# ioloizou/g1_locomotion

Hardware: AMD Instinct MI355X
Metric: QP solves/sec, SRBD N=10 12-state/12-input (higher is better)
Workload: dtype f64; 1 GPU; configs[1]: batch=4096/GPU random SRBD states, N=10, 2-contact alternating single support friction cone, fp64; tails deferred (SRBDQP_FLAG_DEFER_TAIL: the ~4 % of a batch that reach a rho-restart mark finish in the next launch on their stream; srbdqp_flush inside the timed region, every batch complete when the clock stops); steps rotate over 4 distinct device batches; horizon=10, batch_per_gpu=4096, kernel=wave_defer_f64_n10_s2, streams=2, longest_first_hint=False, deferred_tails=True, world_size=1, distinct_batches=4, max_iter=250, rho_restart_iter=0, rho_restart_count=0, set_up_dtype=f64

## Files before the change

### g1_locomotion_amd/csrc/srbdqp_admm.hpp

```cpp
#pragma once
#include "srbdqp_common.hpp"

namespace srbdqp {

#ifdef SRBDQP_PROFILE_ADMM
#define ADMM_T(var) do { unsigned long long t_; asm volatile("s_memtime %0\n\ts_waitcnt lgkmcnt(0)" : "=s"(t_) :: "memory"); var = (long long)t_; } while (0)
#else
#define ADMM_T(var) do { } while (0)
#endif

__device__ __forceinline__ double dpp_swap1(double v) {
    int lo = __double2loint(v), hi = __double2hiint(v);
    lo = __builtin_amdgcn_update_dpp(lo, lo, 0xB1, 0xF, 0xF, false);
    hi = __builtin_amdgcn_update_dpp(hi, hi, 0xB1, 0xF, 0xF, false);
    return __hiloint2double(hi, lo);
}

__device__ __forceinline__ double dpp_swap2(double v) {
    int lo = __double2loint(v), hi = __double2hiint(v);
    lo = __builtin_amdgcn_update_dpp(lo, lo, 0x4E, 0xF, 0xF, false);
    hi = __builtin_amdgcn_update_dpp(hi, hi, 0x4E, 0xF, 0xF, false);
    return __hiloint2double(hi, lo);
}

__device__ __forceinline__ int wave_next(int v) { return __builtin_amdgcn_update_dpp(0, v, 0x130, 0xF, 0xF, true); }
__device__ __forceinline__ int wave_prev(int v) { return __builtin_amdgcn_update_dpp(0, v, 0x138, 0xF, 0xF, true); }
__device__ __forceinline__ float wave_next(float v) { return __int_as_float(wave_next(__float_as_int(v))); }
__device__ __forceinline__ float wave_prev(float v) { return __int_as_float(wave_prev(__float_as_int(v))); }
__device__ __forceinline__ double wave_next(double v) { return __hiloint2double(wave_next(__double2hiint(v)), wave_next(__double2loint(v))); }
__device__ __forceinline__ double wave_prev(double v) { return __hiloint2double(wave_prev(__double2hiint(v)), wave_prev(__double2loint(v))); }
template <typename T> __device__ __forceinline__ T contact_fz(T v, int ax) { const T n1 = wave_next(v), n2 = wave_next(n1); return (ax == 0) ? n2 : ((ax == 1) ? n1 : v); }
template <typename T> __device__ __forceinline__ T contact_sum_xy(T v) { const T p1 = wave_prev(v), p2 = wave_prev(p1); return p2 + p1; }

typedef unsigned v2u_t __attribute__((ext_vector_type(2)));
__device__ __forceinline__ void row_chunks(int v, int (&ch)[4]) {
    const v2u_t ab = __builtin_amdgcn_permlane32_swap((unsigned)v, (unsigned)v, false, false);
    const v2u_t p = __builtin_amdgcn_permlane16_swap(ab[0], ab[0], false, false);
    const v2u_t q = __builtin_amdgcn_permlane16_swap(ab[1], ab[1], false, false);
    ch[0] = (int)p[0]; ch[1] = (int)p[1]; ch[2] = (int)q[0]; ch[3] = (int)q[1];
}
__device__ __forceinline__ void row_chunks(double v, double (&ch)[4]) {
    int lo[4], hi[4];
    row_chunks(__double2loint(v), lo);
    row_chunks(__double2hiint(v), hi);
#pragma unroll
    for (int c = 0; c < 4; ++c) ch[c] = __hiloint2double(hi[c], lo[c]);
}

__device__ __forceinline__ double bperm_f64(double v, int src_lane) {
    const int lo = __builtin_amdgcn_ds_bpermute(src_lane << 2, __double2loint(v));
    const int hi = __builtin_amdgcn_ds_bpermute(src_lane << 2, __double2hiint(v));
    return __hiloint2double(hi, lo);
}

#define SRBDQP_FD(A, K, J) "v_fmac_f64_dpp %" #A ", %4, %" #K " row_newbcast:" #J " row_mask:0xf bank_mask:0xf\n\t"
#define SRBDQP_FD4(K0, K1, K2, K3, J0, J1, J2, J3) SRBDQP_FD(0, K0, J0) SRBDQP_FD(1, K1, J1) SRBDQP_FD(2, K2, J2) SRBDQP_FD(3, K3, J3)
template <int CNT>
__device__ __forceinline__ void fmac_row_bcast_block(double (&acc)[4], double ch, const double* k) {
    static_assert(CNT == 4 || CNT == 8 || CNT == 12 || CNT == 16, "whole groups of four terms");
    if constexpr (CNT == 4)
        asm volatile("s_nop 1\n\t" SRBDQP_FD4(5, 6, 7, 8, 0, 1, 2, 3)
                     : "+v"(acc[0]), "+v"(acc[1]), "+v"(acc[2]), "+v"(acc[3]) : "v"(ch), "v"(k[0]), "v"(k[1]), "v"(k[2]), "v"(k[3]));
    else if constexpr (CNT == 8)
        asm volatile("s_nop 1\n\t" SRBDQP_FD4(5, 6, 7, 8, 0, 1, 2, 3) SRBDQP_FD4(9, 10, 11, 12, 4, 5, 6, 7)
                     : "+v"(acc[0]), "+v"(acc[1]), "+v"(acc[2]), "+v"(acc[3])
                     : "v"(ch), "v"(k[0]), "v"(k[1]), "v"(k[2]), "v"(k[3]), "v"(k[4]), "v"(k[5]), "v"(k[6]), "v"(k[7]));
    else if constexpr (CNT == 12)
        asm volatile("s_nop 1\n\t" SRBDQP_FD4(5, 6, 7, 8, 0, 1, 2, 3) SRBDQP_FD4(9, 10, 11, 12, 4, 5, 6, 7) SRBDQP_FD4(13, 14, 15, 16, 8, 9, 10, 11)
                     : "+v"(acc[0]), "+v"(acc[1]), "+v"(acc[2]), "+v"(acc[3])
                     : "v"(ch), "v"(k[0]), "v"(k[1]), "v"(k[2]), "v"(k[3]), "v"(k[4]), "v"(k[5]), "v"(k[6]), "v"(k[7]), "v"(k[8]), "v"(k[9]), "v"(k[10]),
                       "v"(k[11]));
    else
        asm volatile("s_nop 1\n\t" SRBDQP_FD4(5, 6, 7, 8, 0, 1, 2, 3) SRBDQP_FD4(9, 10, 11, 12, 4, 5, 6, 7) SRBDQP_FD4(13, 14, 15, 16, 8, 9, 10, 11)
                     SRBDQP_FD4(17, 18, 19, 20, 12, 13, 14, 15)
                     : "+v"(acc[0]), "+v"(acc[1]), "+v"(acc[2]), "+v"(acc[3])
                     : "v"(ch), "v"(k[0]), "v"(k[1]), "v"(k[2]), "v"(k[3]), "v"(k[4]), "v"(k[5]), "v"(k[6]), "v"(k[7]), "v"(k[8]), "v"(k[9]), "v"(k[10]),
                       "v"(k[11]), "v"(k[12]), "v"(k[13]), "v"(k[14]), "v"(k[15]));
}
template <int KS, int C>
struct RowBcastChunk {
    template <int KN>
    static __device__ __forceinline__ void run(double (&acc)[4], double ch, const double (&kin)[KN]) {
        constexpr int CNT = (KS - 16 * C) < 16 ? (KS - 16 * C) : 16;
        if constexpr (CNT > 0) fmac_row_bcast_block<CNT>(acc, ch, kin + 16 * C);
    }
};

template <int CTRL, int ROW_MASK>
__device__ __forceinline__ double dpp_max_step(double v) {
    const int lo = __builtin_amdgcn_update_dpp(0, __double2loint(v), CTRL, ROW_MASK, 0xF, false);
    const int hi = __builtin_amdgcn_update_dpp(0, __double2hiint(v), CTRL, ROW_MASK, 0xF, false);
    return fmax(v, __hiloint2double(hi, lo));
}
__device__ __forceinline__ double wave_max_nonneg(double v) {
    v = dpp_max_step<0x111, 0xF>(v);
    v = dpp_max_step<0x112, 0xF>(v);
    v = dpp_max_step<0x114, 0xF>(v);
    v = dpp_max_step<0x118, 0xF>(v);
    v = dpp_max_step<0x142, 0xA>(v);
    v = dpp_max_step<0x143, 0xC>(v);
    return v;
}

template <int CTRL, int ROW_MASK>
__device__ __forceinline__ float dpp_maxf_step(float v) {
    const int o = __builtin_amdgcn_update_dpp(0, __float_as_int(v), CTRL, ROW_MASK, 0xF, false);
    return fmaxf(v, __int_as_float(o));
}
__device__ __forceinline__ float wave_maxf_nonneg(float v) {
    v = dpp_maxf_step<0x111, 0xF>(v);
    v = dpp_maxf_step<0x112, 0xF>(v);
    v = dpp_maxf_step<0x114, 0xF>(v);
    v = dpp_maxf_step<0x118, 0xF>(v);
    v = dpp_maxf_step<0x142, 0xA>(v);
    v = dpp_maxf_step<0x143, 0xC>(v);
    return v;
}

#define SRBDQP_MAX4(CTRL) "v_max_f32_dpp %0, %0, %0 " CTRL "\n\tv_max_f32_dpp %1, %1, %1 " CTRL "\n\tv_max_f32_dpp %2, %2, %2 " CTRL "\n\tv_max_f32_dpp %3, %3, %3 " CTRL "\n\t"
__device__ __forceinline__ void wave_maxf4_nonneg(float& v0, float& v1, float& v2, float& v3) {
    asm volatile("s_nop 1\n\t"
                 SRBDQP_MAX4("row_shr:1 row_mask:0xf bank_mask:0xf") SRBDQP_MAX4("row_shr:2 row_mask:0xf bank_mask:0xf")
                 SRBDQP_MAX4("row_shr:4 row_mask:0xf bank_mask:0xf") SRBDQP_MAX4("row_shr:8 row_mask:0xf bank_mask:0xf")
                 SRBDQP_MAX4("row_bcast:15 row_mask:0xa bank_mask:0xf") SRBDQP_MAX4("row_bcast:31 row_mask:0xc bank_mask:0xf")
                 : "+v"(v0), "+v"(v1), "+v"(v2), "+v"(v3));
}

}
```

### g1_locomotion_amd/csrc/srbdqp_mfma.hpp

```cpp
#pragma once
#include "srbdqp_common.hpp"
#include "srbdqp_admm.hpp"

namespace srbdqp {

constexpr bool kMfmaReady = true;

#ifdef SRBDQP_PROFILE_F
#define F_T(var) do { unsigned long long t_; asm volatile("s_memtime %0\n\ts_waitcnt lgkmcnt(0)" : "=s"(t_) :: "memory"); var = (long long)t_; } while (0)
#else
#define F_T(var) do { } while (0)
#endif

typedef double v4d __attribute__((ext_vector_type(4)));

__device__ __forceinline__ v4d mfma_f64(double a, double b, v4d c) {
    return __builtin_amdgcn_mfma_f64_16x16x4f64(a, b, c, 0, 0, 0);
}

__device__ __forceinline__ double readlane_f64(double v, int lane) {
    const int lo = __builtin_amdgcn_readlane(__double2loint(v), lane);
    const int hi = __builtin_amdgcn_readlane(__double2hiint(v), lane);
    return __hiloint2double(hi, lo);
}

__device__ __forceinline__ int tile_id(int a, int b) { return (b * (b + 1)) / 2 + a; }

template <bool SWZ>
__device__ __forceinline__ void store_tile(double* tile, const v4d& v, int lane) {
    const int col = lane & 15, g = lane >> 4;
#pragma unroll
    for (int r = 0; r < 4; ++r) {
        const int row = g + 4 * r;
        tile[row * 16 + (SWZ ? (col ^ row) : col)] = v[r];
    }
}

typedef float v4f __attribute__((ext_vector_type(4)));
__device__ __forceinline__ v4d mma16(double a, double b, v4d c) { return __builtin_amdgcn_mfma_f64_16x16x4f64(a, b, c, 0, 0, 0); }
__device__ __forceinline__ v4f mma16(float a, float b, v4f c) { return __builtin_amdgcn_mfma_f32_16x16x4f32(a, b, c, 0, 0, 0); }
template <typename TT> __device__ __forceinline__ int crow(int kq, int q) { return (sizeof(TT) == 8) ? kq + 4 * q : 4 * kq + q; }
template <typename TT, bool SWZ, typename V4>
__device__ __forceinline__ void store_tile_t(TT* tile, const V4& v, int lane) {
    const int col = lane & 15, g = lane >> 4;
#pragma unroll
    for (int q = 0; q < 4; ++q) {
        const int row = crow<TT>(g, q);
        tile[row * 16 + (SWZ ? (col ^ row) : col)] = v[q];
    }
}

__device__ __forceinline__ double fast_rsqrt(double d) {
    const double r = __builtin_amdgcn_rsq(d);
    const double h = 0.5 * d * r;
    return fma(r, fma(-h, r, 0.5), r);
}

__device__ __forceinline__ double fast_rsqrt2(double d) {
    double r = __builtin_amdgcn_rsq(d);
    double h = 0.5 * d * r;
    r = fma(r, fma(-h, r, 0.5), r);
    h = 0.5 * d * r;
    return fma(r, fma(-h, r, 0.5), r);
}

template <int KB>
__device__ __forceinline__ void diag16_block(v4d& s, v4d& rr, v4d& w, double& pmin, int lane) {
    const int col = lane & 15, k = lane >> 4, li = col & 3;
    const double sk = s[KB];
    const double d00 = readlane_f64(sk, 4 * KB), d01 = readlane_f64(sk, 4 * KB + 1), d02 = readlane_f64(sk, 4 * KB + 2), d03 = readlane_f64(sk, 4 * KB + 3);
    const double d11 = readlane_f64(sk, 16 + 4 * KB + 1), d12 = readlane_f64(sk, 16 + 4 * KB + 2), d13 = readlane_f64(sk, 16 + 4 * KB + 3);
    const double d22 = readlane_f64(sk, 32 + 4 * KB + 2), d23 = readlane_f64(sk, 32 + 4 * KB + 3);
    const double d33 = readlane_f64(sk, 48 + 4 * KB + 3);
    const double x00 = fast_rsqrt(d00);
    const double r01 = d01 * x00, r02 = d02 * x00, r03 = d03 * x00;
    const double p1 = fma(-r01, r01, d11);
    const double x11 = fast_rsqrt(p1);
    const double r12 = fma(-r01, r02, d12) * x11, r13 = fma(-r01, r03, d13) * x11;
    const double p2 = fma(-r12, r12, fma(-r02, r02, d22));
    const double x22 = fast_rsqrt(p2);
    const double r23 = fma(-r12, r13, fma(-r02, r03, d23)) * x22;
    const double p3 = fma(-r23, r23, fma(-r13, r13, fma(-r03, r03, d33)));
    const double x33 = fast_rsqrt(p3);
    pmin = (d00 > 0.0 && p1 > 0.0 && p2 > 0.0 && p3 > 0.0) ? pmin : -1.0;
    const double x01 = -x00 * r01 * x11;
    const double x12 = -x11 * r12 * x22;
    const double x23 = -x22 * r23 * x33;
    const double x02 = -fma(x00, r02, x01 * r12) * x22;
    const double x13 = -fma(x11, r13, x12 * r23) * x33;
    const double x03 = -fma(x00, r03, fma(x01, r13, x02 * r23)) * x33;
    const double c0 = x00;
    const double c1 = (k == 0) ? x01 : x11;
    const double c2 = (k == 0) ? x02 : (k == 1) ? x12 : x22;
    const double c3 = (k == 0) ? x03 : (k == 1) ? x13 : (k == 2) ? x23 : x33;
    double a = (li == 0) ? c0 : (li == 1) ? c1 : (li == 2) ? c2 : c3;
    a = (k <= li) ? a : 0.0;
    const v4d zero = (v4d){0.0, 0.0, 0.0, 0.0};
    double u = mfma_f64(a, sk, zero)[KB];
    u = (col >= 4 * KB) ? u : 0.0;
    const double wk = mfma_f64(a, rr[KB], zero)[KB];
    w[KB] = wk;
    if constexpr (KB < 3) {
        s = mfma_f64(-u, u, s);
        const double am = (col >= 4 * (KB + 1)) ? u : 0.0;
        rr = mfma_f64(-am, wk, rr);
        diag16_block<KB + 1>(s, rr, w, pmin, lane);
    }
}

__device__ __forceinline__ v4d diag16_invert_mfma(v4d s, int lane, bool& ok) {
    const int col = lane & 15, g = lane >> 4;
    v4d rr, w;
#pragma unroll
    for (int r = 0; r < 4; ++r) { rr[r] = (g + 4 * r == col) ? 1.0 : 0.0; w[r] = 0.0; }
    double pmin = 1.0e300;
    diag16_block<0>(s, rr, w, pmin, lane);
    ok = pmin > 0.0;
    return w;
}


template <int I>
__device__ __forceinline__ void fmac_newbcast(double& acc, double nu, double m) {
    asm("v_fmac_f64_dpp %0, %1, %2 row_newbcast:%3 row_mask:0xf bank_mask:0xf" : "+v"(acc) : "v"(nu), "v"(m), "n"(I));
}
template <int K>
__device__ __forceinline__ double mov_newbcast(double v) {
    double d;
    asm("s_nop 1\n\tv_mov_b64_dpp %0, %1 row_newbcast:%2 row_mask:0xf bank_mask:0xf" : "=v"(d) : "v"(v), "n"(K));
    return d;
}
template <int K, int I>
struct Diag16Rows {
    static __device__ __forceinline__ void run(double (&S)[16], double (&R)[16], double nu, double u, double wk) {
        if constexpr (I < 16) {
            fmac_newbcast<I>(S[I], nu, u);
            fmac_newbcast<I>(R[I], nu, wk);
            Diag16Rows<K, I + 1>::run(S, R, nu, u, wk);
        }
    }
};
template <int K, int KEND = 16>
__device__ __forceinline__ void diag16_pivot(double (&S)[16], double (&R)[16], bool& ok) {
    const double d = mov_newbcast<K>(S[K]);
    ok = ok && (d > 0.0);
    const double r = fast_rsqrt(d);
    const double u = S[K] * r;
    const double wk = R[K] * r;
    R[K] = wk;
    if constexpr (K < 15) {
        double nu;
        asm("v_mul_f64 %0, %1, %2\n\ts_nop 1" : "=v"(nu) : "v"(S[K]), "v"(-r));
        Diag16Rows<K, K + 1>::run(S, R, nu, u, wk);
    }
    if constexpr (K + 1 < KEND) diag16_pivot<K + 1, KEND>(S, R, ok);
}
__device__ __forceinline__ v4d diag16_invert_dpp(v4d s, int lane, bool& ok, double* tile) {
    const int col = lane & 15, g = lane >> 4;
    asm volatile("" ::: "memory");
#pragma unroll
    for (int r = 0; r < 4; ++r) tile[(g + 4 * r) * 16 + col] = s[r];
    asm volatile("" ::: "memory");
    double S[16], R[16];
#pragma unroll
    for (int i = 0; i < 16; ++i) { S[i] = tile[i * 16 + col]; R[i] = (i == col) ? 1.0 : 0.0; }
    asm volatile("" ::: "memory");
    ok = true;
    diag16_pivot<0>(S, R, ok);
    if (g == 0) {
#pragma unroll
        for (int i = 0; i < 16; ++i) tile[i * 16 + (col ^ i)] = R[i];
    }
    asm volatile("" ::: "memory");
    v4d w;
#pragma unroll
    for (int q = 0; q < 4; ++q) { const int row = g + 4 * q; w[q] = tile[row * 16 + (col ^ row)]; }
    asm volatile("" ::: "memory");
    return w;
}
__device__ __forceinline__ double pk_even_rows(double x) {
    int alo, ahi, blo, bhi;
    asm("v_mov_b32 %0, %4\n\tv_mov_b32 %2, %4\n\tv_mov_b32 %1, %5\n\tv_mov_b32 %3, %5\n\ts_nop 1\n\t"
        "v_permlane16_swap_b32 %0, %2\n\tv_permlane16_swap_b32 %1, %3"
        : "=&v"(alo), "=&v"(ahi), "=&v"(blo), "=&v"(bhi) : "v"(__double2loint(x)), "v"(__double2hiint(x)));
    return __hiloint2double(ahi, alo);
}
#define SRBDQP_PK(P, I) "v_fmac_f64_dpp %" #P ", %8, %9 row_newbcast:" #I " row_mask:0xf bank_mask:0xf\n\t"
#define SRBDQP_PK_LO7 SRBDQP_PK(7, 7)
#define SRBDQP_PK_LO6 SRBDQP_PK(6, 6) SRBDQP_PK_LO7
#define SRBDQP_PK_LO5 SRBDQP_PK(5, 5) SRBDQP_PK_LO6
#define SRBDQP_PK_LO4 SRBDQP_PK(4, 4) SRBDQP_PK_LO5
#define SRBDQP_PK_LO3 SRBDQP_PK(3, 3) SRBDQP_PK_LO4
#define SRBDQP_PK_LO2 SRBDQP_PK(2, 2) SRBDQP_PK_LO3
#define SRBDQP_PK_HI15 SRBDQP_PK(7, 15)
#define SRBDQP_PK_HI14 SRBDQP_PK(6, 14) SRBDQP_PK_HI15
#define SRBDQP_PK_HI13 SRBDQP_PK(5, 13) SRBDQP_PK_HI14
#define SRBDQP_PK_HI12 SRBDQP_PK(4, 12) SRBDQP_PK_HI13
#define SRBDQP_PK_HI11 SRBDQP_PK(3, 11) SRBDQP_PK_HI12
#define SRBDQP_PK_HI10 SRBDQP_PK(2, 10) SRBDQP_PK_HI11
#define SRBDQP_PK_HI9 SRBDQP_PK(1, 9) SRBDQP_PK_HI10
#define SRBDQP_PK_HI8 SRBDQP_PK(0, 8) SRBDQP_PK_HI9
#define SRBDQP_PK_MID11 SRBDQP_PK(3, 11)
#define SRBDQP_PK_MID10 SRBDQP_PK(2, 10) SRBDQP_PK_MID11
#define SRBDQP_PK_MID9 SRBDQP_PK(1, 9) SRBDQP_PK_MID10
#define SRBDQP_PK_MID8 SRBDQP_PK(0, 8) SRBDQP_PK_MID9
#define SRBDQP_PK_ASM(TAIL, B) asm("s_nop 1\n\t" TAIL : "+v"(X[B]), "+v"(X[B + 1]), "+v"(X[B + 2]), "+v"(X[B + 3]), "+v"(X[B + 4]), "+v"(X[B + 5]), "+v"(X[B + 6]), "+v"(X[B + 7]) : "v"(nu), "v"(y))
template <int FROM, int END = 16>
__device__ __forceinline__ void pk_rows(double (&X)[16], double nu, double y) {
    static_assert(END == 16 || END == 12 || END == 8, "whole k-steps of four rows");
    if constexpr (FROM == 2) SRBDQP_PK_ASM(SRBDQP_PK_LO2, 0);
    else if constexpr (FROM == 3) SRBDQP_PK_ASM(SRBDQP_PK_LO3, 0);
    else if constexpr (FROM == 4) SRBDQP_PK_ASM(SRBDQP_PK_LO4, 0);
    else if constexpr (FROM == 5) SRBDQP_PK_ASM(SRBDQP_PK_LO5, 0);
    else if constexpr (FROM == 6) SRBDQP_PK_ASM(SRBDQP_PK_LO6, 0);
    else if constexpr (FROM == 7) SRBDQP_PK_ASM(SRBDQP_PK_LO7, 0);
    if constexpr (END == 8) return;
    else if constexpr (END == 12) {
        if constexpr (FROM <= 8) SRBDQP_PK_ASM(SRBDQP_PK_MID8, 8);
        else if constexpr (FROM == 9) SRBDQP_PK_ASM(SRBDQP_PK_MID9, 8);
        else if constexpr (FROM == 10) SRBDQP_PK_ASM(SRBDQP_PK_MID10, 8);
        else if constexpr (FROM == 11) SRBDQP_PK_ASM(SRBDQP_PK_MID11, 8);
    }
    else if constexpr (FROM <= 8) SRBDQP_PK_ASM(SRBDQP_PK_HI8, 8);
    else if constexpr (FROM == 9) SRBDQP_PK_ASM(SRBDQP_PK_HI9, 8);
    else if constexpr (FROM == 10) SRBDQP_PK_ASM(SRBDQP_PK_HI10, 8);
    else if constexpr (FROM == 11) SRBDQP_PK_ASM(SRBDQP_PK_HI11, 8);
    else if constexpr (FROM == 12) SRBDQP_PK_ASM(SRBDQP_PK_HI12, 8);
    else if constexpr (FROM == 13) SRBDQP_PK_ASM(SRBDQP_PK_HI13, 8);
    else if constexpr (FROM == 14) SRBDQP_PK_ASM(SRBDQP_PK_HI14, 8);
    else if constexpr (FROM == 15) SRBDQP_PK_ASM(SRBDQP_PK_HI15, 8);
}
#undef SRBDQP_PK_ASM
#undef SRBDQP_PK_HI8
#undef SRBDQP_PK_HI9
#undef SRBDQP_PK_HI10
#undef SRBDQP_PK_HI11
#undef SRBDQP_PK_HI12
#undef SRBDQP_PK_HI13
#undef SRBDQP_PK_HI14
#undef SRBDQP_PK_HI15
#undef SRBDQP_PK_MID8
#undef SRBDQP_PK_MID9
#undef SRBDQP_PK_MID10
#undef SRBDQP_PK_MID11
#undef SRBDQP_PK_LO2
#undef SRBDQP_PK_LO3
#undef SRBDQP_PK_LO4
#undef SRBDQP_PK_LO5
#undef SRBDQP_PK_LO6
#undef SRBDQP_PK_LO7
#undef SRBDQP_PK
struct PkTile {
    static constexpr int kIdent = 272;
    static constexpr int kDoubles = kIdent + 256;
    static constexpr __host__ __device__ int wrow(int row) { return 17 * row; }
};
__device__ __forceinline__ void pk_ident_store(double* tile, int lane) {
    const int col = lane & 15, g = lane >> 4;
#pragma unroll
    for (int r = 0; r < 4; ++r) tile[PkTile::kIdent + lane + 64 * r] = (g + 4 * r == col) ? 1.0 : 0.0;
}
template <int K, int NP = 16>
__device__ __forceinline__ void diag16_pivot_packed(double (&X)[16], unsigned& worst) {
    const double sk = pk_even_rows(X[K]);
    const double d = mov_newbcast<K>(sk);
    const unsigned dh = (unsigned)__double2hiint(d) - 1u;
    worst = dh > worst ? dh : worst;
    const double r = fast_rsqrt(d);
    const double y = X[K] * r;
    if constexpr (K + 1 < NP) {
        double nu;
        asm("v_mul_f64 %1, %3, -%4\n\ts_nop 1\n\tv_fmac_f64_dpp %0, %1, %2 row_newbcast:%5 row_mask:0xf bank_mask:0xf"
            : "+v"(X[K + 1]), "=&v"(nu) : "v"(y), "v"(sk), "v"(r), "n"(K + 1));
        if constexpr (K + 2 < NP) pk_rows<K + 2, NP>(X, nu, y);
        X[K] = y;
        diag16_pivot_packed<K + 1, NP>(X, worst);
    } else {
        X[K] = y;
    }
}
template <int NP = 16>
__device__ __forceinline__ v4d diag16_invert_dpp_packed(v4d s, int lane, bool& ok, double* tile) {
    static_assert(NP == 16 || NP == 12 || NP == 8, "padding in whole k-steps of four rows");
    const int col = lane & 15, g = lane >> 4;
    asm volatile("" ::: "memory");
#pragma unroll
    for (int r = 0; r < 4; ++r) tile[lane + 64 * r] = s[r];
    asm volatile("" ::: "memory");
    const double* rowp = tile + col + ((g & 1) ? PkTile::kIdent : 0);
    double X[16];
#pragma unroll
    for (int i = 0; i < 16; ++i) X[i] = rowp[i * 16];
    asm volatile("" ::: "memory");
    unsigned worst = 0u;
    diag16_pivot_packed<0, NP>(X, worst);
    ok = worst < 0x7fefffffu;
    if (g == 1) {
#pragma unroll
        for (int i = 0; i < 16; ++i) tile[PkTile::wrow(i) + col] = X[i];
    }
    asm volatile("" ::: "memory");
    const double* cp = tile + lane + g;
    v4d w;
#pragma unroll
    for (int q = 0; q < 4; ++q) w[q] = cp[PkTile::wrow(4) * q];
    asm volatile("" ::: "memory");
    return w;
}

template <typename TI, typename TO>
__device__ __forceinline__ void diag16_invert_dpp_tiles(const TI* in, TO* out, int lane, bool& ok) {
    const int col = lane & 15, g = lane >> 4;
    double S[16], R[16];
#pragma unroll
    for (int i = 0; i < 16; ++i) { S[i] = (double)in[i * 16 + col]; R[i] = (i == col) ? 1.0 : 0.0; }
    asm volatile("s_waitcnt lgkmcnt(0)" ::: "memory");
    ok = true;
    diag16_pivot<0>(S, R, ok);
    if (g == 0) {
#pragma unroll
        for (int i = 0; i < 16; ++i) out[i * 16 + (col ^ i)] = (TO)R[i];
    }
    asm volatile("" ::: "memory");
}

}
```

### g1_locomotion_amd/csrc/srbdqp_setup1.hpp

```cpp
#pragma once
#include "srbdqp_split.hpp"

namespace srbdqp {

#ifdef SRBDQP_WAVE_STAMPS
#define WSTAMP(a, b, idx) SRBDQP_STAMP(a, b, idx)
#define WSTAMP_RT(a, b, idx) do { if ((a).stamps && threadIdx.x == 0) (a).stamps[(size_t)(b) * 16 + (idx)] = (long long)__builtin_amdgcn_s_memrealtime(); } while (0)
#else
#define WSTAMP(a, b, idx) do { } while (0)
#define WSTAMP_RT(a, b, idx) do { } while (0)
#endif

template <int N, int MAXS>
struct Setup1Smem {
    using S = CompactSmem<N, MAXS>;
    static constexpr int n = Dims<N>::n;
    static constexpr int up2(int v) { return (v + 1) & ~1; }
    static constexpr int o_x0 = S::o_x0, o_tm = S::o_tm, o_J = S::o_J;
    static constexpr int o_cp = S::o_R;
    static constexpr int o_mt = o_cp + up2(9 * N);
    static constexpr int o_ab = o_mt + 18 * N;
    static constexpr int o_gv = o_mt + up2(9 * S::NPAIR);
    static constexpr int o_t1 = o_gv + up2(9 * N);
    static constexpr int o_t2 = o_t1 + up2(9 * N);
// ... 90 lines not shown
            const bool over = lane < N && __popcll((bal >> (4 * (lane < N ? lane : 0))) & 0xFull) > MAXS;
            const unsigned long long viol = __ballot(over);
            if (lane == 0) {
                imisc[0] = __popcll(bal);
                imisc[1] = viol != 0ull;
                sm[S::o_misc] = 0.0;
                sm[S::o_misc + 1] = 0.0;
            }
        }
#pragma unroll
        for (int t = 0; t < JT; ++t) {
            const int tt = lane + 64 * t;
            const int tc = tt < 12 * N ? tt : 0, t3 = (int)((unsigned)tc / 3u), k = t3 >> 2, cc = tt - 12 * k, ax = tc - 3 * t3;
            const double cs = __shfl(yc, k), sn = __shfl(ys, k);
            const double i0 = a.iinv[0], i1 = a.iinv[1], i2 = a.iinv[2];
            const double w00 = cs * cs * i0 + sn * sn * i1, w01 = cs * sn * (i0 - i1), w11 = sn * sn * i0 + cs * cs * i1;
            const double rx = v_f[t][0] - v_p[t][0];
            const double ry = v_f[t][1] - v_p[t][1];
            const double rz = v_f[t][2] - v_p[t][2];
            const double s0 = (ax == 0) ? 0.0 : ((ax == 1) ? -rz : ry);
            const double s1 = (ax == 0) ? rz : ((ax == 1) ? 0.0 : -rx);
            const double s2 = (ax == 0) ? -ry : ((ax == 1) ? rx : 0.0);
            if (tt < 12 * N) {
                double* J = sm + S::o_J + k * 36;
                J[0 * 12 + cc] = w00 * s0 + w01 * s1;
                J[1 * 12 + cc] = w01 * s0 + w11 * s1;
                J[2 * 12 + cc] = i2 * s2;
            }
        }
    }
    static_assert(N <= 16, "the prefix chain stays inside one 16-lane DPP row");
    double ccm = 0.0 + yc, csm = 0.0 + ys;
#pragma unroll
    for (int k = 1; k < N; ++k) {
        ccm = row_prev(ccm) + yc;
        csm = row_prev(csm) + ys;
    }
    if (lane < N) {
        double* C = sm + L1::o_cp + lane * 9;
        C[0] = ccm;  C[1] = csm; C[2] = 0.0;
        C[3] = -csm; C[4] = ccm; C[5] = 0.0;
        C[6] = 0.0;  C[7] = 0.0; C[8] = (double)(lane + 1);
    }
    __syncthreads();
    const int na = imisc[0];
    const int n_eff = 3 * na;
    double* xs0 = sm + L1::o_mt;
    static_assert(L1::o_end - L1::o_mt >= n + 12 * N, "early-exit scratch");
    if (RP != 2 && (imisc[1] != 0 || na == 0)) {
        if constexpr (DUMP) { if (lane == 0) a.ub_out[(size_t)b * m] = (imisc[1] != 0) ? -1.0 : 0.0; return false; }
        for (int c = lane; c < n; c += 64) xs0[c] = 0.0;
        if (io.y_out) for (int i = lane; i < m; i += 64) io.y_out[(size_t)b * m + i] = 0.0;
        if (lane == 0) {
            if (io.status) io.status[b] = (imisc[1] != 0) ? kStatusContactBound : 1;
            if (io.iters) io.iters[b] = a.iters_base;
            if constexpr (!FUSED) ws[S::o_misc + 1] = 1.0;
        }
        __syncthreads();
        rollout_and_store_to<N, S, 64>(a, io.u_out, io.x_out, b, sm, xs0, xs0 + n);
        return false;
    }

    WSTAMP(a, b, 1);
    const double dt = a.dt, dt2 = a.dt * a.dt, dtm = a.dt * a.inv_mass, dt2m = dt2 * a.inv_mass;
    double* DE = sm + L1::o_mt;
    double* GV = sm + L1::o_gv;
    if constexpr (RP != 2) {
#pragma unroll
        for (int t = 0; t < JT; ++t) {
            const int k = lane + 64 * t;
            const int kc = k < n ? k : 0, i = kc / 12, kk = kc - 12 * i;
            const double v = SQ[kk] * (free_response_sel<N, L1>(a, sm, i, kk) - v_xr[t]);
            if (k < n) sm[L1::o_eh + k] = v;
        }
    }
    const int pair_c = lane < L1::kPairs ? lane : L1::kPairs - 1;
    const int pair_r = pair_c / (N + 1), pair_k = pair_c - pair_r * (N + 1);
    const bool pair_lo = pair_k < N - pair_r;
    const int pair_m = pair_lo ? pair_r : N - 1 - pair_r, pair_i = pair_m + (pair_lo ? pair_k : pair_k - (N - pair_r));
    const double pair_da = CP[9 * pair_i] - CP[9 * pair_m], pair_db = CP[9 * pair_i + 1] - CP[9 * pair_m + 1];
    double* PD = sm + L1::o_pd;
    double* PQ = sm + L1::o_pq;
    {
        const double w0 = SQ[0] * SQ[0], w1 = SQ[1] * SQ[1], w2 = SQ[2] * SQ[2];
        const double da = pair_da, db = pair_db, dz = (double)(pair_i - pair_m);
        if (lane < L1::kPairs) {
            PD[2 * lane] = da;
            PD[2 * lane + 1] = db;
            PQ[4 * lane] = fma(w0 * da, da, (w1 * db) * db);
            PQ[4 * lane + 1] = fma(w0 * da, db, -((w1 * db) * da));
            PQ[4 * lane + 2] = fma(w0 * db, db, (w1 * da) * da);
            PQ[4 * lane + 3] = (pair_i == N - 1) ? 0.0 : (w2 * dz) * dz;
        }
    }
    __syncthreads();
    const int pair_base = (2 * lane < N) ? lane * (N + 1) : (N - lane) * N;
    if (lane < N) {
        const int mm = lane;
        double t1a = 0.0, t1b = 0.0, t2aa = 0.0, t2ab = 0.0, t2bb = 0.0, t2zz = 0.0;
#pragma unroll
        for (int s = 0; s < N; ++s) {
            if (s < N - mm) {
                const double* pd = PD + 2 * (pair_base + s);
                const double* pq = PQ + 4 * (pair_base + s);
                t1a += pd[0];
                t1b += pd[1];
                t2aa += pq[0];
                t2ab += pq[1];
                t2bb += pq[2];
                t2zz += pq[3];
            }
        }
        const double dzl = (double)(N - 1 - mm);
        t2zz = fma((SQ[2] * SQ[2]) * dzl, dzl, t2zz);
        const double t1z = (double)(((N - mm) * (N - mm - 1)) / 2);
        const double Cm[9] = {ccm, csm, 0.0, -csm, ccm, 0.0, 0.0, 0.0, (double)(mm + 1)};
        const double t1[9] = {t1a, t1b, 0.0, -t1b, t1a, 0.0, 0.0, 0.0, t1z};
        const double t2[9] = {t2aa, t2ab, 0.0, t2ab, t2bb, 0.0, 0.0, 0.0, t2zz};
        de_step<N>(Cm, t1, t2, SQ, dt2, mm, DE + 18 * mm);
    }
    auto gt_tables = [&](const double* vec) {
        {
            const double* v = vec + 12 * pair_i;
            const double p0 = SQ[0] * v[0], p1 = SQ[1] * v[1], p2 = SQ[2] * v[2], dz = (double)(pair_i - pair_m);
            if (lane < L1::kPairs) {
                PQ[4 * lane] = fma(dt, SQ[6] * v[6], dt2 * fma(pair_da, p0, (-pair_db) * p1));
                PQ[4 * lane + 1] = fma(dt, SQ[7] * v[7], dt2 * fma(pair_db, p0, pair_da * p1));
                PQ[4 * lane + 2] = fma(dt, SQ[8] * v[8], dt2 * (dz * p2));
            }
        }
        __syncthreads();
        if (lane < 3 * N) {
            const int j = lane / 3, comp = lane - 3 * j;
            const double* pq = PQ + 4 * ((2 * j < N) ? j * (N + 1) : (N - j) * N) + comp;
            double acc = 0.0;
#pragma unroll
            for (int s = 0; s < N; ++s)
                if (s < N - j) acc += pq[4 * s];
            GV[9 * j + comp] = acc;
        }
        static_assert(6 * N <= 64, "the force entries of the G'v tables are one trip of the wave");
        if (lane < 6 * N) {
            const int j = lane / 6, comp = 3 + (lane - 6 * j);
            const double* v = vec + 12 * j + ((comp < 6) ? comp : 3 + comp);
            const double winc = (comp < 6) ? 1.0 : 0.0;
            double acc = 0.0, w = (comp < 6) ? 0.0 : 1.0;
#pragma unroll
            for (int s = 0; s < N; ++s) {
                if (s < N - j) {
                    double term = w * v[12 * s];
                    asm volatile("" : "+v"(term));
                    acc += term;
                }
                w += winc;
            }
            GV[9 * j + comp] = acc;
        }
    };
    auto gt_eval = [&](int c) -> double {
        const int e = c / 3, ax = c - 3 * e, gc = act[e], j = gc >> 2;
        const double* J = sm + S::o_J + j * 36 + 3 * (gc & 3) + ax;
        const double* g = GV + 9 * j;
        return a.s * (J[0] * g[0] + J[12] * g[1] + J[24] * g[2] + SQ[3 + ax] * dt2m * g[3 + ax] + SQ[9 + ax] * dtm * g[6 + ax]);
    };
    __syncthreads();
    if constexpr (RP != 2) gt_tables(sm + L1::o_eh);
    __syncthreads();
    WSTAMP(a, b, 2);
    if constexpr (RP != 2) for (int c = lane; c < n_eff; c += 64) sm[S::o_q + c] = gt_eval(c);
    if (RP >= 2 || a.warm_u) {
        double* TF = sm + L1::o_tf;
        for (int c = lane; c < n_eff; c += 64)
            sm[L1::o_x0c + c] = (RP >= 2 ? park[c] : a.warm_u[(size_t)b * n + 3 * act[c / 3] + (c % 3)]) / a.s;
        __syncthreads();
        for (int tt = lane; tt < 6 * N; tt += 64) {
            const int j = tt / 6, comp = tt - 6 * j;
            double acc = 0.0;
            for (int e = (j ? icnt[j - 1] : 0); e < icnt[j]; ++e) {
                const double* x = sm + L1::o_x0c + 3 * e;
                if (comp < 3) {
                    const double* J = sm + S::o_J + j * 36 + comp * 12 + 3 * (act[e] & 3);
                    acc += J[0] * x[0] + J[1] * x[1] + J[2] * x[2];
                } else {
                    acc += x[comp - 3];
                }
            }
            TF[tt] = acc;
        }
        __syncthreads();
        for (int k = lane; k < n; k += 64) {
            const int i = k / 12, kk = k - 12 * i;
            const double acc = gx_row<N>(CP, TF, i, kk, dt, dt2, dtm, dt2m);
            sm[L1::o_gx + k] = SQ[kk] * a.s * acc;
        }
        __syncthreads();
        gt_tables(sm + L1::o_gx);
        __syncthreads();
        for (int c = lane; c < n_eff; c += 64) sm[S::o_px0 + c] = gt_eval(c) + a.rs2 * sm[L1::o_x0c + c];
    } else {
        for (int c = lane; c < n_eff; c += 64) sm[S::o_px0 + c] = 0.0;
    }

    if constexpr (PHI) {
        double* phi = ws + W::o_phi;
        const double x0_keep = (lane < 13) ? sm[S::o_x0 + lane] : 0.0;
        for (int kc = 0; kc < 13; ++kc) {
            __syncthreads();
            if (lane < 13) sm[S::o_x0 + lane] = (lane == kc) ? 1.0 : 0.0;
            __syncthreads();
            for (int k = lane; k < n; k += 64) {
                const int i = k / 12, kk = k - 12 * i;
                sm[L1::o_eh + k] = SQ[kk] * free_response<N, L1>(a, sm, i, kk);
            }
            __syncthreads();
            gt_tables(sm + L1::o_eh);
            __syncthreads();
            for (int c = lane; c < n_eff; c += 64) phi[c * 13 + kc] = gt_eval(c);
        }
        __syncthreads();
        if (lane < 13) sm[S::o_x0 + lane] = x0_keep;
        __syncthreads();
    }
    WSTAMP(a, b, 3);
    v4d Kt[NT][NT];
    __syncthreads();
    {
        double* AB = sm + L1::o_ab;
        kasm_rows<N>(sm + S::o_J, CP, DE, SQ, act, n_eff, a.s, dt2m, dtm, AB, lane, 64, 16 * NT);
        __syncthreads();
        typedef double d2 __attribute__((ext_vector_type(2)));
        const double dgxy = uni(a.rs2 + a.sigma + 2.0 * rho_b), dgz = uni(a.rs2 + a.sigma + (4.0 * a.mu * a.mu + a.rho_fz) * rho_b);
        const int d3 = (int)((unsigned)(mcol - kq + 3) % 3u);
        const int m3 = (int)((unsigned)mcol % 3u);
        const double ind[3] = {d3 == 0 ? 1.0 : 0.0, d3 == 1 ? 1.0 : 0.0, d3 == 2 ? 1.0 : 0.0};
        double eqd[4];
#pragma unroll
        for (int q = 0; q < 4; ++q) eqd[q] = (kq + 4 * q == mcol) ? 1.0 : 0.0;
        double Bv[NT][8], dcol[NT];
#pragma unroll
        for (int tb = 0; tb < NT; ++tb) {
            const int c = 16 * tb + mcol;
            const d2* row = reinterpret_cast<const d2*>(AB + kAbStride * c + 8);
#pragma unroll
            for (int i = 0; i < 4; ++i) { const d2 v = row[i]; Bv[tb][2 * i] = v[0]; Bv[tb][2 * i + 1] = v[1]; }
            dcol[tb] = (c < n_eff) ? ((m3 != (5 - tb % 3) % 3) ? dgxy : dgz) : 1.0;
        }
#pragma unroll
        for (int ta = 0; ta < NT; ++ta) {
#pragma unroll
            for (int q = 0; q < 4; ++q) {
                const int r = 16 * ta + kq + 4 * q;
                const d2* row = reinterpret_cast<const d2*>(AB + kAbStride * r);
                double Av[8];
#pragma unroll
                for (int i = 0; i < 4; ++i) { const d2 v = row[i]; Av[2 * i] = v[0]; Av[2 * i + 1] = v[1]; }
#pragma unroll
                for (int tb = ta; tb < NT; ++tb) {
                    double v = Av[0] * Bv[tb][0];
#pragma unroll
                    for (int i = 1; i < 6; ++i) v = fma(Av[i], Bv[tb][i], v);
                    const double ft = fma(Av[7], Bv[tb][7], Av[6] * Bv[tb][6]);
                    v = fma(ind[((ta + q - tb) % 3 + 3) % 3], ft, v);
                    if (ta == tb) v = fma(eqd[q], dcol[tb], v);
                    Kt[ta][tb][q] = v;
                }
            }
        }
    }
    __syncthreads();
    WSTAMP(a, b, 4);
    WSTAMP(a, b, 5);
    if constexpr (DUMP) {
        dump_presolved<N>(a, b, n_eff, na, sm + S::o_q, act, [&](auto&& put) {
#pragma unroll
            for (int ta = 0; ta < NT; ++ta)
#pragma unroll
                for (int tb = ta; tb < NT; ++tb)
#pragma unroll
                    for (int q = 0; q < 4; ++q)
                        if (16 * ta + kq + 4 * q <= 16 * tb + mcol) put(16 * ta + kq + 4 * q, 16 * tb + mcol, Kt[ta][tb][q]);
        });
        return false;
    }

    double* scr = sm + L1::o_scr;
    pk_ident_store(scr, lane);
    const double* const wop = scr + PkTile::wrow(mcol) + kq;
    auto a_operand_read = [&](double (&op)[4]) {
#pragma unroll
        for (int r = 0; r < 4; ++r) op[r] = wop[4 * r];
        asm volatile("" ::: "memory");
    };
    const v4d zero4 = (v4d){0.0, 0.0, 0.0, 0.0};
    constexpr int PAD = 16 * NT - W::KS;
    static_assert(PAD >= 0 && PAD < 16, "KS ends inside the last tile");
    constexpr int kLastSteps = 4 - PAD / 4;
    constexpr int kLastPivots = 16 - 4 * (PAD / 4);

    bool all_ok = true;
#pragma unroll
    for (int j = 0; j < NT; ++j) {
        bool ok;
        const v4d w = (j == NT - 1) ? diag16_invert_dpp_packed<kLastPivots>(Kt[j][j], lane, ok, scr)
                                    : diag16_invert_dpp_packed(Kt[j][j], lane, ok, scr);
        all_ok = all_ok && ok;
        if (j + 1 < NT) {
            double wa[4];
            a_operand_read(wa);
#pragma unroll
            for (int bb = j + 1; bb < NT; ++bb) {
                v4d o = zero4;
#pragma unroll
                for (int r = 0; r < 4; ++r) o = mfma_f64(wa[r], Kt[j][bb][r], o);
                Kt[j][bb] = o;
            }
#pragma unroll
            for (int aa = j + 1; aa < NT; ++aa)
#pragma unroll
                for (int bb = aa; bb < NT; ++bb)
#pragma unroll
                    for (int r = 0; r < 4; ++r) Kt[aa][bb] = mfma_f64(-Kt[j][aa][r], Kt[j][bb][r], Kt[aa][bb]);
#pragma unroll
            for (int l = j + 1; l < NT; ++l) {
                v4d o = zero4;
#pragma unroll
                for (int r = 0; r < 4; ++r) o = mfma_f64(-Kt[j][l][r], w[r], o);
                Kt[j][l] = o;
            }
        }
        v4d pj = zero4;
#pragma unroll
        for (int r = 0; r < (j == NT - 1 ? kLastSteps : 4); ++r) pj = mfma_f64(w[r], w[r], pj);
        Kt[j][j] = pj;
    }
    if (!all_ok && lane == 0) sm[S::o_misc] = 1.0;
    WSTAMP(a, b, 6);
    WSTAMP(a, b, 7);

    double kin[W::KS];
    {
        if constexpr (!FUSED) {
            for (int i = lane; i < S::o_R; i += 64) ws[i] = sm[i];
        }
        double* stg = sm + L1::o_cp;
        static_assert(L1::o_end - L1::o_cp >= NT * L1::kStgTile, "staging of one block column of K^-1");
        [[maybe_unused]] double* kinv = FUSED ? nullptr : ws + W::o_kinv;
        [[maybe_unused]] const int grp = lane >> 4;
        v4d Ku[NT][NT];
#pragma unroll
        for (int cb = NT - 1; cb >= 0; --cb) {
            v4d Xc[NT];
            asm volatile("" ::: "memory");
#pragma unroll
            for (int l = cb + 1; l < NT; ++l)
#pragma unroll
                for (int q = 0; q < 4; ++q) stg[l * L1::kStgTile + mcol * L1::kStgRow + kq + 4 * q] = Ku[cb][l][q];
            asm volatile("" ::: "memory");
#pragma unroll
            for (int l = cb + 1; l < NT; ++l)
#pragma unroll
                for (int q = 0; q < 4; ++q) Xc[l][q] = stg[l * L1::kStgTile + (kq + 4 * q) * L1::kStgRow + mcol];
            asm volatile("" ::: "memory");
#pragma unroll
            for (int g = cb; g >= 0; --g) {
                v4d o = (g == cb) ? Kt[cb][cb] : zero4;
#pragma unroll
                for (int l = g + 1; l < NT; ++l)
#pragma unroll
                    for (int r = 0; r < (l == NT - 1 ? kLastSteps : 4); ++r) o = mfma_f64(Kt[g][l][r], Xc[l][r], o);
                Xc[g] = o;
                if (g < cb) Ku[g][cb] = o;
                if constexpr (FUSED) {
#pragma unroll
                    for (int q = 0; q < 4; ++q) stg[g * L1::kStgTile + (kq + 4 * q) * L1::kStgRow + mcol] = o[q];
                } else {
                    const int col = 16 * cb + mcol;
#pragma unroll
                    for (int q = 0; q < 4; ++q) {
                        const int row = 16 * g + kq + 4 * q;
                        if (row < n_eff && col < W::KS) kinv[row * W::KS + col] = (col < n_eff) ? o[q] : 0.0;
                        if (g != cb && col < n_eff && row < W::KS) kinv[col * W::KS + row] = (row < n_eff) ? o[q] : 0.0;
                    }
                }
            }
            if constexpr (FUSED) {
                asm volatile("" ::: "memory");
                const double2* rowp = reinterpret_cast<const double2*>(stg + grp * L1::kStgTile + mcol * L1::kStgRow);
#pragma unroll
                for (int h = 0; h < 8; ++h) {
                    if (16 * cb + 2 * h + 1 < W::KS + 1) {
                        const double2 v = rowp[h];
                        if (16 * cb + 2 * h < W::KS) kin[16 * cb + 2 * h] = v.x;
                        if (16 * cb + 2 * h + 1 < W::KS) kin[16 * cb + 2 * h + 1] = v.y;
                    }
                }
                asm volatile("" ::: "memory");
            }
        }
    }
    if constexpr (FUSED) {
        if (__builtin_amdgcn_readfirstlane(n_eff) < W::KS) {
#pragma unroll
            for (int c = 0; c < W::KS; ++c) kin[c] = (lane < n_eff && c < n_eff) ? kin[c] : 0.0;
        }
        __syncthreads();
        WSTAMP(a, b, 8);
        WSTAMP(a, b, 9);
        static_assert(L1::o_end >= SplitSmem<N, MAXS>::o_end, "the ADMM body's vectors live in this kernel's LDS");
        if constexpr (RP == 0) {
            admm_wave_body<N, MAXS>(a, b, rho_b, sm, kin);
        } else {
            WaveRestart rs;
            const int left = a.max_iter - rs_done;
            rs.pass = rs_pass;
            rs.more = rs_pass < a.restart_max && a.restart_every < left;
            rs.kcap = rs.more ? a.restart_every : left;
            rs.park = park;
            int status = -1, iters = 0;
            admm_wave_iterations<N, MAXS, true>(a, io, RP == 1 ? a.warm_u : nullptr, RP == 1 ? a.warm_y : nullptr, b, rho_b, sm, kin, sm + SplitSmem<N, MAXS>::o_xs,
                                                status, iters, &rs);
            rs_done += iters;
            if (status == 2 && rs.more) {
                rho_b = restart_rho_of(rho_b, rs.v);
                ++rs_pass;
                __syncthreads();
                return true;
            }
            admm_wave_finish<N, MAXS>(a, io, b, sm, status, rs_done);
        }
        WSTAMP(a, b, 10);
        WSTAMP(a, b, 11);
        WSTAMP_RT(a, b, 13);
    }
    return false;
}

template <int N, int MAXS, bool FUSED, bool DUMP = false, bool PHI = false, bool RST = false>
__global__ __launch_bounds__(64, 2) void srbdqp_setup1_kernel(KArgs a) {
    static_assert(!(PHI && FUSED), "dq/dx0 is a hand-over of the split pipeline");
    static_assert(!RST || (FUSED && !DUMP), "the restart in place belongs to the fused solve");
    static_assert(Setup1Smem<N, MAXS>::supported, "one wave holds all tiles: at most 4 x 4 tiles");
    static_assert(4 * N <= 64, "one ballot compacts the contact flags");
    extern __shared__ __attribute__((aligned(16))) double sm[];
    if ((int)blockIdx.x >= a.B) return;
    if (a.count_ptr && (int)blockIdx.x >= *a.count_ptr) return;
    const int b = SRBDQP_QP_INDEX(a);
    if (SRBDQP_RESTART_SKIP(a, b)) return;
    double rho_b = SRBDQP_RHO_OF(a, b);
    int rs_pass = 0, rs_done = 0;
    const QpIo io = io_of(a);
    if constexpr (!RST) {
        setup1_pass<N, MAXS, FUSED, DUMP, PHI, 0>(a, io, b, sm, rho_b, rs_pass, rs_done);
    } else {
        bool again = setup1_pass<N, MAXS, FUSED, DUMP, PHI, 1>(a, io, b, sm, rho_b, rs_pass, rs_done);
        if (!again) return;
        again = setup1_pass<N, MAXS, FUSED, DUMP, PHI, 2>(a, io, b, sm, rho_b, rs_pass, rs_done);
        if (!again) return;
        again = setup1_pass<N, MAXS, FUSED, DUMP, PHI, 2>(a, io, b, sm, rho_b, rs_pass, rs_done);
        if (!again) return;
        KArgs al = a;
        al.restart_max = 0;
        setup1_pass<N, MAXS, FUSED, DUMP, PHI, 2>(al, io, b, sm, rho_b, rs_pass, rs_done);
    }
}

__device__ __forceinline__ unsigned long long unis_u64(unsigned long long v) {
    int lo, hi;
    asm volatile("s_nop 1\n\tv_readfirstlane_b32 %0, %2\n\tv_readfirstlane_b32 %1, %3" : "=s"(lo), "=s"(hi) : "v"((int)(unsigned)v), "v"((int)(unsigned)(v >> 32)));
    return ((unsigned long long)(unsigned)hi << 32) | (unsigned long long)(unsigned)lo;
}
template <typename T> __device__ __forceinline__ T* unis_ptr(T* p) { return reinterpret_cast<T*>(unis_u64(reinterpret_cast<unsigned long long>(p))); }

__device__ __forceinline__ double* tail_claim(const KArgs& a) {
    int slot = 0;
    if (threadIdx.x == 0) slot = atomicAdd(a.tail_cnt + a.tail_iout, 1);
    slot = __builtin_amdgcn_readfirstlane(slot);
    if (slot >= a.tail_cap) return nullptr;
    return reinterpret_cast<double*>(a.tail_lists) + ((size_t)a.tail_iout * (size_t)a.tail_cap + (size_t)slot) * kTailRecDoubles;
}

__device__ __forceinline__ bool tail_export(const KArgs& a, const QpIo& io, int b, double rho_b, int rs_pass, int rs_done, const double* park) {
    const int lane = threadIdx.x;
    double* rec = tail_claim(a);
    if (!rec) return false;
    if (lane == 0) {
        TailRecHead* hd = reinterpret_cast<TailRecHead*>(rec);
        hd->b = b; hd->pass = rs_pass; hd->done = rs_done; hd->pad = 0; hd->rho = rho_b; hd->io = io;
        if (io.status) io.status[b] = kStatusPending;
    }
    rec[16 + lane] = park[lane]; rec[80 + lane] = park[64 + lane]; rec[144 + lane] = park[128 + lane];
    return true;
}

template <int N, int MAXS, bool FLUSH = false>
__global__ __launch_bounds__(64, 2) void srbdqp_wave_defer_kernel(KArgs a) {
    static_assert(Setup1Smem<N, MAXS>::supported && 4 * N <= 64, "the one-wave kernel's limits");
    extern __shared__ __attribute__((aligned(16))) double sm[];
    using L1 = Setup1Smem<N, MAXS>;
    const int lane = threadIdx.x;
    const int T = a.tail_wgs;
    double* const park = sm + L1::o_end;
    auto in_place = [&](const QpIo& io, const int b, double rho_b, int rs_pass, int rs_done) __attribute__((always_inline)) {
        bool again = setup1_pass<N, MAXS, true, false, false, 2>(a, io, b, sm, rho_b, rs_pass, rs_done);
        if (!again) return;
        again = setup1_pass<N, MAXS, true, false, false, 2>(a, io, b, sm, rho_b, rs_pass, rs_done);
        if (!again) return;
        KArgs al = a;
        al.restart_max = 0;
        setup1_pass<N, MAXS, true, false, false, 2>(al, io, b, sm, rho_b, rs_pass, rs_done);
    };
    if ((int)blockIdx.x < T) {
        const int i = blockIdx.x;
        int cnt = a.tail_cnt[a.tail_iin];
        cnt = cnt < a.tail_cap ? cnt : a.tail_cap;
        if (i == 0 && lane == 0) a.tail_cnt[a.tail_izero] = 0;
        const double* lin = reinterpret_cast<const double*>(a.tail_lists) + (size_t)a.tail_iin * (size_t)a.tail_cap * kTailRecDoubles;
        if (i >= cnt) return;
        const double* rec = lin + (size_t)i * kTailRecDoubles;
        const TailRecHead* hd = reinterpret_cast<const TailRecHead*>(rec);
        QpIo io;
        io.x0 = unis_ptr(hd->io.x0); io.xref = unis_ptr(hd->io.xref); io.foot = unis_ptr(hd->io.foot); io.pcom = unis_ptr(hd->io.pcom);
        io.contact = unis_ptr(hd->io.contact); io.u_out = unis_ptr(hd->io.u_out); io.x_out = unis_ptr(hd->io.x_out); io.y_out = unis_ptr(hd->io.y_out);
        io.status = unis_ptr(hd->io.status); io.iters = unis_ptr(hd->io.iters);
        const int b = __builtin_amdgcn_readfirstlane(hd->b);
        int rs_pass = __builtin_amdgcn_readfirstlane(hd->pass), rs_done = __builtin_amdgcn_readfirstlane(hd->done);
        double rho_b = unis(hd->rho);
        park[lane] = rec[16 + lane]; park[64 + lane] = rec[80 + lane]; park[128 + lane] = rec[144 + lane];
        __syncthreads();
        if (!setup1_pass<N, MAXS, true, false, false, 3>(a, io, b, sm, rho_b, rs_pass, rs_done)) return;
        if constexpr (!FLUSH) { if (tail_export(a, io, b, rho_b, rs_pass, rs_done, park)) return; }
        in_place(io, b, rho_b, rs_pass, rs_done);
    } else if constexpr (!FLUSH) {
        const int wg = (int)blockIdx.x - T;
        if (wg >= a.B) return;
        const int b = a.perm ? a.perm[wg] : wg;
        double rho_b = a.rho_qp ? a.rho_qp[b] : a.rho;
        int rs_pass = 0, rs_done = 0;
        const QpIo io = io_of(a);
        if (!setup1_pass<N, MAXS, true, false, false, 1>(a, io, b, sm, rho_b, rs_pass, rs_done)) return;
        if (tail_export(a, io, b, rho_b, rs_pass, rs_done, park)) return;
        in_place(io, b, rho_b, rs_pass, rs_done);
    }
}

}
```

Measured before the change: 43.97 million QP/s.

## Ride the first off-diagonal panel through the diagonal pivot and use 64-bit permlane moves

The blocked Cholesky/inverse in setup now lets the first off-diagonal tile (Kt[j][j+1]) pass through the packed DPP pivot sweep on the otherwise idle lane group 3. This removes the separate MFMA multiply of that tile by the inverted diagonal block. It costs extra LDS scratch (a new panel region) plus more stores and loads per pivot. Separately, the f64 row_chunks and pk_even_rows helpers now copy operands with v_mov_b64 and call the permlane swap builtins on both halves, which should cut the number of 32-bit moves and swaps.

```diff
diff --git a/g1_locomotion_amd/csrc/srbdqp_admm.hpp b/g1_locomotion_amd/csrc/srbdqp_admm.hpp
--- a/g1_locomotion_amd/csrc/srbdqp_admm.hpp
+++ b/g1_locomotion_amd/csrc/srbdqp_admm.hpp
@@ -40,11 +40,19 @@
     ch[0] = (int)p[0]; ch[1] = (int)p[1]; ch[2] = (int)q[0]; ch[3] = (int)q[1];
 }
 __device__ __forceinline__ void row_chunks(double v, double (&ch)[4]) {
-    int lo[4], hi[4];
-    row_chunks(__double2loint(v), lo);
-    row_chunks(__double2hiint(v), hi);
-#pragma unroll
-    for (int c = 0; c < 4; ++c) ch[c] = __hiloint2double(hi[c], lo[c]);
+    double c;
+    asm("v_mov_b64 %0, %1\n\ts_nop 1" : "=&v"(c) : "v"(v));
+    const v2u_t lo = __builtin_amdgcn_permlane32_swap((unsigned)__double2loint(v), (unsigned)__double2loint(c), false, false);
+    const v2u_t hi = __builtin_amdgcn_permlane32_swap((unsigned)__double2hiint(v), (unsigned)__double2hiint(c), false, false);
+    const double a = __hiloint2double((int)hi[0], (int)lo[0]), b = __hiloint2double((int)hi[1], (int)lo[1]);
+    double a2, b2;
+    asm("v_mov_b64 %0, %2\n\tv_mov_b64 %1, %3\n\ts_nop 1" : "=&v"(a2), "=&v"(b2) : "v"(a), "v"(b));
+    const v2u_t plo = __builtin_amdgcn_permlane16_swap((unsigned)__double2loint(a), (unsigned)__double2loint(a2), false, false);
+    const v2u_t phi = __builtin_amdgcn_permlane16_swap((unsigned)__double2hiint(a), (unsigned)__double2hiint(a2), false, false);
+    const v2u_t qlo = __builtin_amdgcn_permlane16_swap((unsigned)__double2loint(b), (unsigned)__double2loint(b2), false, false);
+    const v2u_t qhi = __builtin_amdgcn_permlane16_swap((unsigned)__double2hiint(b), (unsigned)__double2hiint(b2), false, false);
+    ch[0] = __hiloint2double((int)phi[0], (int)plo[0]); ch[1] = __hiloint2double((int)phi[1], (int)plo[1]);
+    ch[2] = __hiloint2double((int)qhi[0], (int)qlo[0]); ch[3] = __hiloint2double((int)qhi[1], (int)qlo[1]);
 }
 
 __device__ __forceinline__ double bperm_f64(double v, int src_lane) {
diff --git a/g1_locomotion_amd/csrc/srbdqp_mfma.hpp b/g1_locomotion_amd/csrc/srbdqp_mfma.hpp
--- a/g1_locomotion_amd/csrc/srbdqp_mfma.hpp
+++ b/g1_locomotion_amd/csrc/srbdqp_mfma.hpp
@@ -179,11 +179,11 @@
     return w;
 }
 __device__ __forceinline__ double pk_even_rows(double x) {
-    int alo, ahi, blo, bhi;
-    asm("v_mov_b32 %0, %4\n\tv_mov_b32 %2, %4\n\tv_mov_b32 %1, %5\n\tv_mov_b32 %3, %5\n\ts_nop 1\n\t"
-        "v_permlane16_swap_b32 %0, %2\n\tv_permlane16_swap_b32 %1, %3"
-        : "=&v"(alo), "=&v"(ahi), "=&v"(blo), "=&v"(bhi) : "v"(__double2loint(x)), "v"(__double2hiint(x)));
-    return __hiloint2double(ahi, alo);
+    double a, b;
+    asm("v_mov_b64 %0, %2\n\tv_mov_b64 %1, %2\n\ts_nop 1" : "=&v"(a), "=&v"(b) : "v"(x));
+    const v2u_t lo = __builtin_amdgcn_permlane16_swap((unsigned)__double2loint(a), (unsigned)__double2loint(b), false, false);
+    const v2u_t hi = __builtin_amdgcn_permlane16_swap((unsigned)__double2hiint(a), (unsigned)__double2hiint(b), false, false);
+    return __hiloint2double((int)hi[0], (int)lo[0]);
 }
 #define SRBDQP_PK(P, I) "v_fmac_f64_dpp %" #P ", %8, %9 row_newbcast:" #I " row_mask:0xf bank_mask:0xf\n\t"
 #define SRBDQP_PK_LO7 SRBDQP_PK(7, 7)
@@ -252,9 +252,11 @@
 #undef SRBDQP_PK
 struct PkTile {
     static constexpr int kIdent = 272;
-    static constexpr int kDoubles = kIdent + 256;
+    static constexpr int kPanel = kIdent + 256;
+    static constexpr int kDoubles = kPanel + 272;
     static constexpr __host__ __device__ int wrow(int row) { return 17 * row; }
 };
+static_assert(PkTile::kIdent % 32 == 16 && PkTile::kPanel % 32 == 16 && PkTile::kIdent >= PkTile::wrow(15) + 16 && PkTile::kDoubles >= PkTile::kPanel + PkTile::wrow(15) + 16, "PkTile");
 __device__ __forceinline__ void pk_ident_store(double* tile, int lane) {
     const int col = lane & 15, g = lane >> 4;
 #pragma unroll
@@ -279,15 +281,20 @@
         X[K] = y;
     }
 }
-template <int NP = 16>
-__device__ __forceinline__ v4d diag16_invert_dpp_packed(v4d s, int lane, bool& ok, double* tile) {
+template <int NP = 16, bool RIDE = false>
+__device__ __forceinline__ v4d diag16_invert_dpp_packed(v4d s, int lane, bool& ok, double* tile, [[maybe_unused]] v4d* panel = nullptr) {
     static_assert(NP == 16 || NP == 12 || NP == 8, "padding in whole k-steps of four rows");
+    static_assert(!RIDE || NP == 16, "the riding panel goes through every pivot");
     const int col = lane & 15, g = lane >> 4;
     asm volatile("" ::: "memory");
 #pragma unroll
     for (int r = 0; r < 4; ++r) tile[lane + 64 * r] = s[r];
-    asm volatile("" ::: "memory");
-    const double* rowp = tile + col + ((g & 1) ? PkTile::kIdent : 0);
+    if constexpr (RIDE) {
+#pragma unroll
+        for (int r = 0; r < 4; ++r) tile[PkTile::kPanel + lane + 64 * r] = (*panel)[r];
+    }
+    asm volatile("" ::: "memory");
+    const double* rowp = tile + col + (RIDE ? (g == 1 ? PkTile::kIdent : g == 3 ? PkTile::kPanel : 0) : ((g & 1) ? PkTile::kIdent : 0));
     double X[16];
 #pragma unroll
     for (int i = 0; i < 16; ++i) X[i] = rowp[i * 16];
@@ -295,15 +302,27 @@
     unsigned worst = 0u;
     diag16_pivot_packed<0, NP>(X, worst);
     ok = worst < 0x7fefffffu;
-    if (g == 1) {
-#pragma unroll
-        for (int i = 0; i < 16; ++i) tile[PkTile::wrow(i) + col] = X[i];
+    if constexpr (RIDE) {
+        if (g & 1) {
+            double* const outp = tile + col + (g == 3 ? PkTile::kPanel : 0);
+#pragma unroll
+            for (int i = 0; i < 16; ++i) outp[PkTile::wrow(i)] = X[i];
+        }
+    } else {
+        if (g == 1) {
+#pragma unroll
+            for (int i = 0; i < 16; ++i) tile[PkTile::wrow(i) + col] = X[i];
+        }
     }
     asm volatile("" ::: "memory");
     const double* cp = tile + lane + g;
     v4d w;
 #pragma unroll
     for (int q = 0; q < 4; ++q) w[q] = cp[PkTile::wrow(4) * q];
+    if constexpr (RIDE) {
+#pragma unroll
+        for (int q = 0; q < 4; ++q) (*panel)[q] = cp[PkTile::kPanel + PkTile::wrow(4) * q];
+    }
     asm volatile("" ::: "memory");
     return w;
 }
diff --git a/g1_locomotion_amd/csrc/srbdqp_setup1.hpp b/g1_locomotion_amd/csrc/srbdqp_setup1.hpp
--- a/g1_locomotion_amd/csrc/srbdqp_setup1.hpp
+++ b/g1_locomotion_amd/csrc/srbdqp_setup1.hpp
@@ -416,17 +416,19 @@
     for (int j = 0; j < NT; ++j) {
         bool ok;
         const v4d w = (j == NT - 1) ? diag16_invert_dpp_packed<kLastPivots>(Kt[j][j], lane, ok, scr)
-                                    : diag16_invert_dpp_packed(Kt[j][j], lane, ok, scr);
+                                    : diag16_invert_dpp_packed<16, true>(Kt[j][j], lane, ok, scr, &Kt[j][j + 1 < NT ? j + 1 : j]);
         all_ok = all_ok && ok;
         if (j + 1 < NT) {
-            double wa[4];
-            a_operand_read(wa);
-#pragma unroll
-            for (int bb = j + 1; bb < NT; ++bb) {
-                v4d o = zero4;
-#pragma unroll
-                for (int r = 0; r < 4; ++r) o = mfma_f64(wa[r], Kt[j][bb][r], o);
-                Kt[j][bb] = o;
+            if (j + 2 < NT) {
+                double wa[4];
+                a_operand_read(wa);
+#pragma unroll
+                for (int bb = j + 2; bb < NT; ++bb) {
+                    v4d o = zero4;
+#pragma unroll
+                    for (int r = 0; r < 4; ++r) o = mfma_f64(wa[r], Kt[j][bb][r], o);
+                    Kt[j][bb] = o;
+                }
             }
 #pragma unroll
             for (int aa = j + 1; aa < NT; ++aa)
```

Result: faster. 44.52 million QP/s (median of 6 runs) (+1.3%).
